# zuds-survey/zuds-pipeline

Hardware: AMD Instinct MI355X
Metric: Mpix/s resample->coadd->subtract, 3072x3072 frames (higher is better)
Workload: dtype f32; 1 GPU; configs[1]+[2]: 32x 3072x3072 TPV frames/GPU, mesh background + weight rescale + Lanczos-3 resample + WEIGHTED coadd (+ AND mask coadd, int16 masks); then 1 science frame/GPU: align ref, hotpants 3x3 regions x 10x10 stamps, r=10, ko=4, subtract; frames_per_gpu=32, size=3072, mask_dtype=int16, combine=WEIGHTED, subtract=True

## Files before the change

zuds-pipeline_amd/csrc/hotpants.hip:

```cpp
#include "hp_dev.h"
#include <sched.h>
#include "chol_diag.h"

static __device__ __forceinline__ void hp_zero_words(int* __restrict__ zero0, int nzero0, int* __restrict__ zero1, int nzero1) {
    if (blockIdx.x != 0) return;
    if (zero0) for (int k = threadIdx.x; k < nzero0; k += blockDim.x) zero0[k] = 0;
    if (zero1) for (int k = threadIdx.x; k < nzero1; k += blockDim.x) zero1[k] = 0;
}
__global__ void k_hp_valid(const float* __restrict__ sci, const float* __restrict__ ref,
                           const uint8_t* __restrict__ bpm, int64_t n, float il, float iu,
                           float tl, float tu, uint8_t* __restrict__ bad,
                           const double* __restrict__ lim, double nsig,
                           int* __restrict__ zero0 = nullptr, int nzero0 = 0,
                           int* __restrict__ zero1 = nullptr, int nzero1 = 0) {
    int64_t p = (int64_t)blockIdx.x * blockDim.x + threadIdx.x;
    hp_zero_words(zero0, nzero0, zero1, nzero1);
    if (lim) {
        il = (float)(lim[0] - nsig * lim[1]);
        tl = (float)(lim[3] - nsig * lim[4]);
    }
    if (p >= n) return;
    float s = sci[p], t = ref[p];
    bool ok = (s == s) && (t == t) && fabsf(s) < 3e38f && fabsf(t) < 3e38f;
    ok = ok && s >= il && s <= iu && t >= tl && t <= tu;
// ... 67 lines not shown
        if (lane == 0) wsum[4 * c + wave] = __popcll(m);
    }
    if (tid == 0) ra_pre[0] = 0;
    __syncthreads();
    {
        const int v = tid < 4 * nch ? wsum[tid] : 0;
        int inc = v;
#pragma unroll
        for (int o = 1; o < 64; o <<= 1) {
            const int t = __shfl_up(inc, o);
            if (lane >= o) inc += t;
        }
        if (lane == 63) wtot[wave] = inc;
        __syncthreads();
        int off = inc - v;
        for (int w = 0; w < wave; ++w) off += wtot[w];
        if (tid < 4 * nch) wsum[tid] = off;
    }
    __syncthreads();
    for (int c = 0; c < nch; ++c) {
        const int x = 256 * c + tid;
        if (x < nx) ra_pre[x + 1] += wsum[4 * c + wave];
    }
    __syncthreads();
    for (int x = tid; x < nx; x += 256) {
        const int a1 = max(x - hw1, 0), b1 = min(x + hw1, nx - 1);
        const int a2 = max(x - hw2, 0), b2 = min(x + hw2, nx - 1);
        out1[r0 + x] = (ra_pre[b1 + 1] - ra_pre[a1]) > 0;
        out2[r0 + x] = (ra_pre[b2 + 1] - ra_pre[a2]) > 0;
    }
}

#define HP_COLSTRIP 96
__global__ __launch_bounds__(256) void k_hp_colany(const uint8_t* __restrict__ in, int nx, int ny, int hw,
                                                   int edge, uint8_t* __restrict__ out) {
    const int x = blockIdx.x * blockDim.x + threadIdx.x;
    const int y0 = blockIdx.y * HP_COLSTRIP, y1 = min(y0 + HP_COLSTRIP, ny);
    if (x >= nx) return;
    int cnt = 0;
    for (int j = max(y0 - hw, 0); j <= min(y0 + hw, ny - 1); ++j) cnt += in[(size_t)j * nx + x] ? 1 : 0;
    for (int y = y0; y < y1; ++y) {
        uint8_t v = cnt > 0;
        if (edge && (x < hw || x >= nx - hw || y < hw || y >= ny - hw)) v = 1;
        out[(size_t)y * nx + x] = v;
        const int add = y + 1 + hw, sub = y - hw;
        if (add < ny) cnt += in[(size_t)add * nx + x] ? 1 : 0;
        if (sub >= 0) cnt -= in[(size_t)sub * nx + x] ? 1 : 0;
    }
}

#define HP_COLSTRIP4 32
__global__ __launch_bounds__(256) void k_hp_colany4(const uint8_t* __restrict__ in, int nx, int ny, int hw,
                                                    int edge, uint8_t* __restrict__ out) {
    const int x = (blockIdx.x * blockDim.x + threadIdx.x) * 4;
    const int y0 = blockIdx.y * HP_COLSTRIP4, y1 = min(y0 + HP_COLSTRIP4, ny);
    if (x >= nx) return;
    const unsigned* in4 = reinterpret_cast<const unsigned*>(in + x);
    const size_t pitch = (size_t)nx / 4;
    auto nz = [](unsigned w, int k) -> int { return ((w >> (8 * k)) & 0xffu) ? 1 : 0; };
    int cnt[4] = {0, 0, 0, 0};
    {
        const int j0 = max(y0 - hw, 0), j1 = min(y0 + hw, ny - 1);
        for (int jb = j0; jb <= j1; jb += 8) {
            unsigned w[8];
#pragma unroll
            for (int u = 0; u < 8; ++u) w[u] = (jb + u <= j1) ? in4[(size_t)(jb + u) * pitch] : 0u;
#pragma unroll
            for (int u = 0; u < 8; ++u)
#pragma unroll
                for (int k = 0; k < 4; ++k) cnt[k] += nz(w[u], k);
        }
    }
    for (int yb = y0; yb < y1; yb += 8) {
        unsigned wa[8], ws[8];
#pragma unroll
        for (int u = 0; u < 8; ++u) {
            const int add = yb + u + 1 + hw, sub = yb + u - hw;
            wa[u] = (add < ny) ? in4[(size_t)add * pitch] : 0u;
            ws[u] = (sub >= 0) ? in4[(size_t)sub * pitch] : 0u;
        }
#pragma unroll
        for (int u = 0; u < 8; ++u) {
            const int y = yb + u;
            if (y < y1) {
                unsigned o = 0;
#pragma unroll
                for (int k = 0; k < 4; ++k) {
                    unsigned v = cnt[k] > 0;
                    if (edge && (x + k < hw || x + k >= nx - hw || y < hw || y >= ny - hw)) v = 1;
                    o |= v << (8 * k);
                }
                *reinterpret_cast<unsigned*>(out + (size_t)y * nx + x) = o;
            }
#pragma unroll
            for (int k = 0; k < 4; ++k) cnt[k] += nz(wa[u], k) - nz(ws[u], k);
        }
    }
}

__global__ __launch_bounds__(256) void k_hp_cells(const hp_plan P, const float* __restrict__ ref,
                                                  const uint8_t* __restrict__ bad,
                                                  const uint8_t* __restrict__ dirty,
                                                  int2* __restrict__ centres) {
    __shared__ double red[4];
    __shared__ float bval[4];
    __shared__ int bidx[4];
    __shared__ int2 chosen[HP_MAXNSS];
    const int cell = blockIdx.x, tid = threadIdx.x;
    const int r = cell / P.ncellr, c = cell - r * P.ncellr;
    const int sy = c / P.nsx, sx = c - sy * P.nsx;
    const int cw = (P.rx1[r] - P.rx0[r]) / P.nsx, ch = (P.ry1[r] - P.ry0[r]) / P.nsy;
    const int cx0 = P.rx0[r] + sx * cw, cy0 = P.ry0[r] + sy * ch;
    const int n = cw * ch;
    double m = 0.0, s = 0.0;
    for (int pass = 0; pass < 4; ++pass) {
        double s0 = 0, s1 = 0;
        for (int k = tid; k < n; k += 256) {
            int yy = k / cw, xx = k - yy * cw;
            size_t idx = (size_t)(cy0 + yy) * P.nx + cx0 + xx;
            if (bad[idx]) continue;
            double v = ref[idx];
            if (pass == 0 || fabs(v - m) <= 3.0 * s) { s0 += 1.0; s1 += v; }
        }
        s0 = block_sum256(s0, red);
        s1 = block_sum256(s1, red);
        if (s0 < 1.0) break;
        double mn = s1 / s0;
        double s2 = 0;
        for (int k = tid; k < n; k += 256) {
            int yy = k / cw, xx = k - yy * cw;
            size_t idx = (size_t)(cy0 + yy) * P.nx + cx0 + xx;
            if (bad[idx]) continue;
            double v = ref[idx];
            if (pass == 0 || fabs(v - m) <= 3.0 * s) s2 += (v - mn) * (v - mn);
        }
        s2 = block_sum256(s2, red);
        m = mn;
        s = sqrt(s2 / s0);
    }
    const double thr = m + P.ft * s;
    for (int k = 0; k < P.nss; ++k) {
        float best = -__builtin_inff();
        int bi = 0x7fffffff;
        for (int q = tid; q < n; q += 256) {
            int yy = q / cw, xx = q - yy * cw;
            int x = cx0 + xx, y = cy0 + yy;
            size_t idx = (size_t)y * P.nx + x;
            if (dirty[idx]) continue;
            float v = ref[idx];
            if (!((double)v >= thr)) continue;
            bool excl = false;
            for (int e = 0; e < k; ++e)
                excl |= (abs(x - chosen[e].x) <= P.hwss) && (abs(y - chosen[e].y) <= P.hwss);
            if (excl) continue;
            if (v > best || (v == best && q < bi)) { best = v; bi = q; }
        }
#pragma unroll
        for (int o = 32; o >= 1; o >>= 1) {
            float ov = __shfl_xor(best, o);
            int oi = __shfl_xor(bi, o);
            if (ov > best || (ov == best && oi < bi)) { best = ov; bi = oi; }
        }
        __syncthreads();
        if ((tid & 63) == 0) { bval[tid >> 6] = best; bidx[tid >> 6] = bi; }
        __syncthreads();
        if (tid == 0) {
            for (int w = 1; w < 4; ++w)
                if (bval[w] > best || (bval[w] == best && bidx[w] < bi)) { best = bval[w]; bi = bidx[w]; }
            int2 cc = make_int2(-1, -1);
            if (bi != 0x7fffffff) { int yy = bi / cw; cc = make_int2(cx0 + bi - yy * cw, cy0 + yy); }
            chosen[k] = cc;
            centres[cell * P.nss + k] = cc;
        }
        __syncthreads();
        if (chosen[k].x < 0) {
            if (tid == 0)
                for (int e = k + 1; e < P.nss; ++e) centres[cell * P.nss + e] = make_int2(-1, -1);
            break;
        }
    }
}

#define HC_PX 24
#define HC_THREADS 512
__global__ __launch_bounds__(HC_THREADS, 4) void k_hp_cells_reg(const hp_plan P, const float* __restrict__ ref,
                                                      const uint8_t* __restrict__ bad,
                                                      const uint8_t* __restrict__ dirty,
                                                      int2* __restrict__ centres) {
    __shared__ double red[HC_THREADS / 64];
    __shared__ float bval[HC_THREADS / 64];
    __shared__ int bidx[HC_THREADS / 64];
    __shared__ int2 chosen[HP_MAXNSS];
    const int cell = blockIdx.x, tid = threadIdx.x;
    const int r = cell / P.ncellr, c = cell - r * P.ncellr;
    const int sy = c / P.nsx, sx = c - sy * P.nsx;
    const int cw = (P.rx1[r] - P.rx0[r]) / P.nsx, ch = (P.ry1[r] - P.ry0[r]) / P.nsy;
    const int cx0 = P.rx0[r] + sx * cw, cy0 = P.ry0[r] + sy * ch;
    const int n = cw * ch;
    const int dyy = HC_THREADS / cw, dxx = HC_THREADS - dyy * cw;
    const int yy0 = tid / cw, xx0 = tid - yy0 * cw;
    float v[HC_PX];
    unsigned long long okm = 0, cleanm = 0;
    {
        int yy = yy0, xx = xx0;
#pragma unroll
        for (int i = 0; i < HC_PX; ++i) {
            const int k = tid + HC_THREADS * i;
            float val = 0.f;
            if (k < n) {
                const size_t idx = (size_t)(cy0 + yy) * P.nx + cx0 + xx;
                val = ref[idx];
                if (!bad[idx]) okm |= 1ull << i;
                if (!dirty[idx]) cleanm |= 1ull << i;
            }
            v[i] = val;
            xx += dxx; yy += dyy;
            if (xx >= cw) { xx -= cw; ++yy; }
        }
    }
    double m = 0.0, s = 0.0;
    for (int pass = 0; pass < 4; ++pass) {
        double s0 = 0, s1 = 0;
#pragma unroll
        for (int i = 0; i < HC_PX; ++i) {
            float vf = v[i];
            asm volatile("" : "+v"(vf));
            const double vv = vf;
            if ((okm >> i & 1) && (pass == 0 || fabs(vv - m) <= 3.0 * s)) { s0 += 1.0; s1 += vv; }
        }
        s0 = block_sum_waves<HC_THREADS / 64>(s0, red);
        s1 = block_sum_waves<HC_THREADS / 64>(s1, red);
        if (s0 < 1.0) break;
        const double mn = s1 / s0;
        double s2 = 0;
#pragma unroll
        for (int i = 0; i < HC_PX; ++i) {
            float vf = v[i];
            asm volatile("" : "+v"(vf));
            const double vv = vf;
            if ((okm >> i & 1) && (pass == 0 || fabs(vv - m) <= 3.0 * s)) s2 += (vv - mn) * (vv - mn);
        }
        s2 = block_sum_waves<HC_THREADS / 64>(s2, red);
        m = mn;
        s = sqrt(s2 / s0);
    }
    const double thr = m + P.ft * s;
    unsigned long long cand = 0;
#pragma unroll
    for (int i = 0; i < HC_PX; ++i)
        if ((cleanm >> i & 1) && ((double)v[i] >= thr)) cand |= 1ull << i;
    int2 last = make_int2(-1000000, -1000000);
    for (int k = 0; k < P.nss; ++k) {
        float best = -__builtin_inff();
        int bi = 0x7fffffff;
        {
            int yy = yy0, xx = xx0;
            asm volatile("" : "+v"(yy), "+v"(xx));
#pragma unroll
            for (int i = 0; i < HC_PX; ++i) {
                if (cand >> i & 1) {
                    const int x = cx0 + xx, y = cy0 + yy, q = tid + HC_THREADS * i;
                    const bool excl = (abs(x - last.x) <= P.hwss) && (abs(y - last.y) <= P.hwss);
                    if (excl) cand &= ~(1ull << i);
                    else if (v[i] > best || (v[i] == best && q < bi)) { best = v[i]; bi = q; }
                }
                xx += dxx; yy += dyy;
                if (xx >= cw) { xx -= cw; ++yy; }
            }
        }
#pragma unroll
        for (int o = 32; o >= 1; o >>= 1) {
            float ov = __shfl_xor(best, o);
            int oi = __shfl_xor(bi, o);
            if (ov > best || (ov == best && oi < bi)) { best = ov; bi = oi; }
        }
        __syncthreads();
        if ((tid & 63) == 0) { bval[tid >> 6] = best; bidx[tid >> 6] = bi; }
        __syncthreads();
        if (tid == 0) {
            for (int w = 1; w < HC_THREADS / 64; ++w)
                if (bval[w] > best || (bval[w] == best && bidx[w] < bi)) { best = bval[w]; bi = bidx[w]; }
            int2 cc = make_int2(-1, -1);
            if (bi != 0x7fffffff) { int yy = bi / cw; cc = make_int2(cx0 + bi - yy * cw, cy0 + yy); }
            chosen[k] = cc;
            centres[cell * P.nss + k] = cc;
        }
        __syncthreads();
        last = chosen[k];
        if (last.x < 0) {
            if (tid == 0)
                for (int e = k + 1; e < P.nss; ++e) centres[cell * P.nss + e] = make_int2(-1, -1);
            break;
        }
    }
}


typedef double double4_t __attribute__((ext_vector_type(4)));

#define GR_KT 32
#define GR_PITCH 34

#define GR_SPLIT 8
static __device__ __forceinline__ void hp_gram_body(const hp_plan& P, const double* __restrict__ X,
                                                 const int* __restrict__ need,
                                                 const int* __restrict__ active,
                                                 double* __restrict__ Gp, const int* __restrict__ guard,
                                                 const int* __restrict__ list) {
    if (guard && *guard == 0) return;
    __shared__ double L[HP_MAXX * GR_PITCH];
    const int tid = threadIdx.x;
    const int ncl = list ? list[0] : (int)gridDim.x;
#pragma unroll 1
    for (int ci = blockIdx.x; ci < ncl; ci += gridDim.x) {
    const int cell = list ? list[1 + ci] : ci;
    __syncthreads();
    if (!need[cell] || active[cell] < 0) continue;
    const double* Xc = X + (size_t)cell * P.nX * P.npixp;
    const int wave = tid >> 6, lane = tid & 63;
    const int li = lane & 15, lk = lane >> 4;
    const int ntile = P.npixp / GR_KT;
    const int per = (ntile + GR_SPLIT - 1) / GR_SPLIT;
    const int kbeg = blockIdx.y * per * GR_KT, kend = min((int)(blockIdx.y + 1) * per, ntile) * GR_KT;
    double4_t acc[4];
#pragma unroll
    for (int c = 0; c < 4; ++c) acc[c] = (double4_t){0.0, 0.0, 0.0, 0.0};
    constexpr int GR_LD = HP_MAXX * GR_KT / 256;
    double nxt[GR_LD];
    auto fetch = [&](int k0) {
#pragma unroll
        for (int q = 0; q < GR_LD; ++q) {
            const int e = tid + 256 * q, row = e >> 5, col = e & 31;
            nxt[q] = row < P.nX ? Xc[(size_t)row * P.npixp + k0 + col] : 0.0;
        }
    };
    if (kbeg < kend) fetch(kbeg);
    for (int k0 = kbeg; k0 < kend; k0 += GR_KT) {
        __syncthreads();
#pragma unroll
        for (int q = 0; q < GR_LD; ++q) {
            const int e = tid + 256 * q, row = e >> 5, col = e & 31;
            L[row * GR_PITCH + col] = nxt[q];
        }
        __syncthreads();
        if (k0 + GR_KT < kend) fetch(k0 + GR_KT);
#pragma unroll
        for (int kk = 0; kk < GR_KT / 4; ++kk) {
            double a = L[(16 * wave + li) * GR_PITCH + 4 * kk + lk];
#pragma unroll
            for (int c = 0; c < 4; ++c) {
                double b = L[(16 * c + li) * GR_PITCH + 4 * kk + lk];
                acc[c] = __builtin_amdgcn_mfma_f64_16x16x4f64(a, b, acc[c], 0, 0, 0);
            }
        }
    }
    double* Gc = Gp + ((size_t)cell * GR_SPLIT + blockIdx.y) * HP_MAXX * HP_MAXX;
#pragma unroll
    for (int c = 0; c < 4; ++c)
#pragma unroll
        for (int rg = 0; rg < 4; ++rg)
            Gc[(size_t)(16 * wave + lk + 4 * rg) * HP_MAXX + 16 * c + li] = acc[c][rg];
    }
}

#define GS_THREADS 1024
static __device__ __forceinline__ void hp_gram_sum_body(const double* __restrict__ Gp,
                                                     const int* __restrict__ need,
                                                     const int* __restrict__ active,
                                                     double* __restrict__ G, const int* __restrict__ guard,
                                                     double* __restrict__ Gold, const int* __restrict__ list) {
    if (guard && *guard == 0) return;
    const int ncl = list ? list[0] : (int)gridDim.x;
    constexpr int NE = HP_MAXX * HP_MAXX / GS_THREADS;
#pragma unroll 1
    for (int ci = blockIdx.x; ci < ncl; ci += gridDim.x) {
        const int cell = list ? list[1 + ci] : ci;
        if (!need[cell] || active[cell] < 0) continue;
        const double* src = Gp + (size_t)cell * GR_SPLIT * HP_MAXX * HP_MAXX;
        double* dst = G + (size_t)cell * HP_MAXX * HP_MAXX;
        double* old = Gold ? Gold + (size_t)cell * HP_MAXX * HP_MAXX : nullptr;
        double part[NE][GR_SPLIT], prev[NE];
#pragma unroll
        for (int q = 0; q < NE; ++q) {
            const int e = threadIdx.x + GS_THREADS * q;
#pragma unroll
            for (int sl = 0; sl < GR_SPLIT; ++sl) part[q][sl] = src[(size_t)sl * HP_MAXX * HP_MAXX + e];
            prev[q] = old ? dst[e] : 0.0;
        }
#pragma unroll
        for (int q = 0; q < NE; ++q) {
            const int e = threadIdx.x + GS_THREADS * q;
            double v = 0.0;
#pragma unroll
            for (int sl = 0; sl < GR_SPLIT; ++sl) v += part[q][sl];
            if (old) old[e] = prev[q];
            dst[e] = v;
        }
    }
}

__device__ inline void col_decode(const hp_plan& P, int c, int* n, int* p) {
    if (c == 0) { *n = 0; *p = -1; return; }
    int k = c - 1;
    if (k < (P.nc - 1) * P.nkp) { *n = 1 + k / P.nkp; *p = k % P.nkp; return; }
    *n = P.nc + (k - (P.nc - 1) * P.nkp);
    *p = -1;
}

__global__ __launch_bounds__(256) void k_hp_build(const hp_plan P, const double* __restrict__ G,
                                                  const double* __restrict__ phi,
                                                  const int* __restrict__ active,
                                                  const int* __restrict__ chg, int sign,
                                                  double* __restrict__ A,
                                                  double* __restrict__ rhs, const int* __restrict__ guard,
                                                  unsigned* __restrict__ zero = nullptr, int nzero = 0) {
    if (guard && *guard == 0) return;
    const int reg = blockIdx.z;
    if (zero && blockIdx.x == 0 && blockIdx.y == 0)
        for (int k = threadIdx.x; k < nzero; k += 256) zero[(size_t)reg * nzero + k] = 0u;
    const int c1 = blockIdx.y * 16 + (threadIdx.x >> 4), c2 = blockIdx.x * 16 + (threadIdx.x & 15);
    if (blockIdx.x > blockIdx.y) return;
    if (c1 >= P.nunk || c2 >= P.nunk) return;
    int n1, p1, n2, p2;
    col_decode(P, c1, &n1, &p1);
    col_decode(P, c2, &n2, &p2);
    double acc = 0.0, racc = 0.0;
    const bool do_rhs = (c2 == 0);
    bool any = false;
    const int* list = chg + P.ncell + reg * (P.ncellr + 1);
    const int ncand = (sign == 0) ? P.ncellr : list[0];
    for (int s0 = 0; s0 < ncand; s0 += 8) {
        double g[8], gr[8], w1[8], w2[8];
        bool on[8];
#pragma unroll
        for (int u = 0; u < 8; ++u) {
            const int s = s0 + u;
            on[u] = false;
            g[u] = gr[u] = 0.0;
            w1[u] = w2[u] = 1.0;
            if (s < ncand) {
                const int cell = (sign == 0) ? reg * P.ncellr + s : list[1 + s];
                on[u] = !(active[cell] < 0 && sign >= 0);
                if (on[u]) {
                    const double* Gc = G + (size_t)cell * HP_MAXX * HP_MAXX;
                    const double* ph = phi + (size_t)cell * P.nkp;
                    if (p1 >= 0) w1[u] = ph[p1];
                    if (p2 >= 0) w2[u] = ph[p2];
                    g[u] = Gc[n1 * HP_MAXX + n2];
                    if (do_rhs) gr[u] = Gc[n1 * HP_MAXX + P.nE];
                }
            }
        }
#pragma unroll
        for (int u = 0; u < 8; ++u)
            if (on[u]) {
                any = true;
                acc += w1[u] * w2[u] * g[u];
                if (do_rhs) racc += w1[u] * gr[u];
            }
    }
    const size_t ia = (size_t)reg * (size_t)(P.nunk + 1) * P.nunk + (size_t)c1 * P.nunk + c2;
    if (sign == 0) {
        if (c2 <= c1) A[ia] = acc;
        if (do_rhs) rhs[(size_t)reg * P.nunk + c1] = racc;
    } else if (any) {
        if (c2 <= c1) A[ia] += sign * acc;
        if (do_rhs) rhs[(size_t)reg * P.nunk + c1] += sign * racc;
    }
}

#define BB_CH 128
#define HBB_PAIRS 5
#define BU_CH 32
#define BB_LDS (BB_CH * 18 + BB_CH / 2)
static __device__ __forceinline__ void hp_pair_decode(const int pair, int* n1o, int* n2o) {
    int n1 = (int)((sqrtf(8.f * (float)pair + 1.f) - 1.f) * 0.5f);
    while (n1 * (n1 + 1) / 2 > pair) --n1;
    while ((n1 + 1) * (n1 + 2) / 2 <= pair) ++n1;
    *n1o = n1;
    *n2o = pair - n1 * (n1 + 1) / 2;
}
static __device__ __forceinline__ void hp_blk_entry_add(const double w1, const double w2, const double g, const double gr,
                                                     const bool do_rhs, double& acc, double& racc) {
    acc += w1 * w2 * g;
    if (do_rhs) racc += w1 * gr;
}
static __device__ __forceinline__ void hp_build_blk_body(const int reg, const int pair, const hp_plan& P, const double* __restrict__ G,
                                                      const double* __restrict__ phi,
                                                      const int* __restrict__ active,
                                                      double* __restrict__ A,
                                                      double* __restrict__ rhs,
                                                      unsigned* __restrict__ zero, int nzero, double* sh) {
    int n1, n2;
    hp_pair_decode(pair, &n1, &n2);
    if (zero && n1 == 0 && n2 == 0)
        for (int k = threadIdx.x; k < nzero; k += 256) zero[(size_t)reg * nzero + k] = 0u;
    const int p1 = threadIdx.x >> 4, p2 = threadIdx.x & 15;
    const bool k1 = n1 >= 1 && n1 < P.nc, k2 = n2 >= 1 && n2 < P.nc;
    const int nk = (P.nc - 1) * P.nkp;
    const int c1 = n1 == 0 ? 0 : (k1 ? 1 + (n1 - 1) * P.nkp + p1 : 1 + nk + (n1 - P.nc));
    const int c2 = n2 == 0 ? 0 : (k2 ? 1 + (n2 - 1) * P.nkp + p2 : 1 + nk + (n2 - P.nc));
    const bool live = p1 < (k1 ? P.nkp : 1) && p2 < (k2 ? P.nkp : 1) && c2 <= c1;
    const bool do_rhs = (c2 == 0);
    double *gs = sh, *grs = sh + BB_CH, *phs = sh + 2 * BB_CH;
    int* ons = reinterpret_cast<int*>(sh + 18 * BB_CH);
    const int tid = threadIdx.x;
    const size_t ia = (size_t)reg * (size_t)(P.nunk + 1) * P.nunk + (size_t)c1 * P.nunk + c2;
    double acc = 0.0, racc = 0.0;
    for (int s0 = 0; s0 < P.ncellr; s0 += BB_CH) {
        const int nch = min(BB_CH, P.ncellr - s0);
        __syncthreads();
        if (tid < nch) {
            const int cell = reg * P.ncellr + s0 + tid;
            const int on = active[cell] >= 0;
            const double* Gc = G + (size_t)cell * HP_MAXX * HP_MAXX;
            ons[tid] = on;
            gs[tid] = on ? Gc[n1 * HP_MAXX + n2] : 0.0;
            grs[tid] = (on && n2 == 0) ? Gc[n1 * HP_MAXX + P.nE] : 0.0;
        }
        for (int e = tid; e < nch * P.nkp; e += 256) {
            const int k = e / P.nkp, pp = e - k * P.nkp;
            phs[k * 16 + pp] = phi[(size_t)(reg * P.ncellr + s0 + k) * P.nkp + pp];
        }
        __syncthreads();
        if (live) {
            for (int k = 0; k < nch; ++k) {
                if (!ons[k]) continue;
                const double w1 = k1 ? phs[k * 16 + p1] : 1.0, w2 = k2 ? phs[k * 16 + p2] : 1.0;
                hp_blk_entry_add(w1, w2, gs[k], do_rhs ? grs[k] : 0.0, do_rhs, acc, racc);
            }
        }
    }
    if (!live) return;
    A[ia] = acc;
    if (do_rhs) rhs[(size_t)reg * P.nunk + c1] = racc;
}

static __device__ __forceinline__ void hp_update_blk_body(const int reg, const int pair0, const hp_plan& P, const double* __restrict__ G,
                                                       const double* __restrict__ phi, const int* __restrict__ active,
                                                       const int* __restrict__ chg, double* __restrict__ A,
                                                       double* __restrict__ rhs, unsigned* __restrict__ zero, int nzero,
                                                       const double* __restrict__ Gold, const double* __restrict__ phiold,
                                                       const int* __restrict__ need, double* sh) {
    static_assert(HBB_PAIRS * BU_CH <= 256 && BU_CH * 16 == 512, "one Gram item and two spatial-term items per thread");
    static_assert(4 * HBB_PAIRS * BU_CH + 2 * BU_CH * 16 + BU_CH <= BB_LDS, "the update's staging fits the build's LDS");
    double (*ug)[HBB_PAIRS][BU_CH] = reinterpret_cast<double (*)[HBB_PAIRS][BU_CH]>(sh);
    double (*ugr)[HBB_PAIRS][BU_CH] = reinterpret_cast<double (*)[HBB_PAIRS][BU_CH]>(sh + 2 * HBB_PAIRS * BU_CH);
    double (*uph)[BU_CH * 16] = reinterpret_cast<double (*)[BU_CH * 16]>(sh + 4 * HBB_PAIRS * BU_CH);
    int* uon = reinterpret_cast<int*>(sh + 4 * HBB_PAIRS * BU_CH + 2 * BU_CH * 16);
    const int tid = threadIdx.x;
    const int npair = P.nE * (P.nE + 1) / 2;
    if (zero && pair0 == 0)
        for (int k = tid; k < nzero; k += 256) zero[(size_t)reg * nzero + k] = 0u;
    const int* list = chg + P.ncell + reg * (P.ncellr + 1);
    const int ncand = list[0];
    if (ncand <= 0) return;
    const int p1 = tid >> 4, p2 = tid & 15;
    const int nk = (P.nc - 1) * P.nkp;
    bool k1[HBB_PAIRS], k2[HBB_PAIRS], live[HBB_PAIRS], do_rhs[HBB_PAIRS], any1[HBB_PAIRS];
    size_t ia[HBB_PAIRS], ir[HBB_PAIRS];
    double av[HBB_PAIRS], rv[HBB_PAIRS], acc0[HBB_PAIRS], racc0[HBB_PAIRS], acc1[HBB_PAIRS], racc1[HBB_PAIRS];
    {
        int n1, n2;
        hp_pair_decode(pair0, &n1, &n2);
#pragma unroll
        for (int q = 0; q < HBB_PAIRS; ++q) {
            k1[q] = n1 >= 1 && n1 < P.nc;
            k2[q] = n2 >= 1 && n2 < P.nc;
            const int c1 = n1 == 0 ? 0 : (k1[q] ? 1 + (n1 - 1) * P.nkp + p1 : 1 + nk + (n1 - P.nc));
            const int c2 = n2 == 0 ? 0 : (k2[q] ? 1 + (n2 - 1) * P.nkp + p2 : 1 + nk + (n2 - P.nc));
            live[q] = pair0 + q < npair && p1 < (k1[q] ? P.nkp : 1) && p2 < (k2[q] ? P.nkp : 1) && c2 <= c1;
            do_rhs[q] = (c2 == 0);
            ia[q] = (size_t)reg * (size_t)(P.nunk + 1) * P.nunk + (size_t)c1 * P.nunk + c2;
            ir[q] = (size_t)reg * P.nunk + c1;
            any1[q] = false;
            av[q] = rv[q] = acc0[q] = racc0[q] = acc1[q] = racc1[q] = 0.0;
            if (live[q]) {
                av[q] = A[ia[q]];
                if (do_rhs[q]) rv[q] = rhs[ir[q]];
            }
            if (++n2 > n1) { ++n1; n2 = 0; }
        }
    }
    const int gq = min(tid / BU_CH, HBB_PAIRS - 1), gk = tid % BU_CH;
    const bool gdo = tid < HBB_PAIRS * BU_CH && pair0 + gq < npair;
    int gn1, gn2;
    hp_pair_decode(min(pair0 + gq, npair - 1), &gn1, &gn2);
    for (int s0 = 0; s0 < ncand; s0 += BU_CH) {
        const int nch = min(BU_CH, ncand - s0);
        __syncthreads();
        {
            const int cg = list[1 + s0 + min(gk, nch - 1)];
            int cp[2], pp[2];
#pragma unroll
            for (int u = 0; u < 2; ++u) {
                const int e = tid + 256 * u;
                cp[u] = list[1 + s0 + min(e >> 4, nch - 1)];
                pp[u] = min(e & 15, P.nkp - 1);
            }
            const int wasg = need[cg], ong = active[cg] >= 0;
            const double* Gn = G + (size_t)cg * HP_MAXX * HP_MAXX;
            const double* Go = Gold + (size_t)cg * HP_MAXX * HP_MAXX;
            const double gnew = Gn[gn1 * HP_MAXX + gn2], gold = Go[gn1 * HP_MAXX + gn2];
            const double rnew = Gn[gn1 * HP_MAXX + P.nE], rold = Go[gn1 * HP_MAXX + P.nE];
            int wasp[2];
            double fnew[2], fold[2];
#pragma unroll
            for (int u = 0; u < 2; ++u) {
                wasp[u] = need[cp[u]];
                fnew[u] = phi[(size_t)cp[u] * P.nkp + pp[u]];
                fold[u] = phiold[(size_t)cp[u] * P.nkp + pp[u]];
            }
            if (gdo && gk < nch) {
                ug[0][gq][gk] = wasg ? gold : gnew;
                ugr[0][gq][gk] = gn2 == 0 ? (wasg ? rold : rnew) : 0.0;
                ug[1][gq][gk] = ong ? gnew : 0.0;
                ugr[1][gq][gk] = (ong && gn2 == 0) ? rnew : 0.0;
                if (gq == 0) uon[gk] = ong;
            }
#pragma unroll
            for (int u = 0; u < 2; ++u) {
                const int e = tid + 256 * u;
                if ((e >> 4) < nch && (e & 15) < P.nkp) {
                    uph[0][e] = wasp[u] ? fold[u] : fnew[u];
                    uph[1][e] = fnew[u];
                }
            }
        }
        __syncthreads();
        for (int k = 0; k < nch; ++k) {
            const double f1o = uph[0][k * 16 + p1], f2o = uph[0][k * 16 + p2];
            const double f1n = uph[1][k * 16 + p1], f2n = uph[1][k * 16 + p2];
            const bool back = uon[k] != 0;
#pragma unroll
            for (int q = 0; q < HBB_PAIRS; ++q)
                if (live[q]) {
                    hp_blk_entry_add(k1[q] ? f1o : 1.0, k2[q] ? f2o : 1.0, ug[0][q][k], do_rhs[q] ? ugr[0][q][k] : 0.0,
                                     do_rhs[q], acc0[q], racc0[q]);
                    if (back) {
                        any1[q] = true;
                        hp_blk_entry_add(k1[q] ? f1n : 1.0, k2[q] ? f2n : 1.0, ug[1][q][k], do_rhs[q] ? ugr[1][q][k] : 0.0,
                                         do_rhs[q], acc1[q], racc1[q]);
                    }
                }
        }
    }
#pragma unroll
    for (int q = 0; q < HBB_PAIRS; ++q)
        if (live[q]) {
            av[q] += -1.0 * acc0[q];
            if (do_rhs[q]) rv[q] += -1.0 * racc0[q];
            if (any1[q]) {
                av[q] += acc1[q];
                if (do_rhs[q]) rv[q] += racc1[q];
            }
            A[ia[q]] = av[q];
            if (do_rhs[q]) rhs[ir[q]] = rv[q];
        }
}

#define BM_CH 128
static __device__ __forceinline__ void hp_build_mfma_body(const hp_plan& P, const double* __restrict__ G,
                                                       const double* __restrict__ phi, const int* __restrict__ active,
                                                       double* __restrict__ A, double* __restrict__ rhs,
                                                       unsigned* __restrict__ zero, int nzero) {
    typedef double bm_double4 __attribute__((ext_vector_type(4)));
// ... 2638 lines not shown
```

zuds-pipeline_amd/csrc/hp_vectors.hip:

```cpp
#include "hp_dev.h"

template <int HWK, bool BIG = false>
static __device__ __forceinline__ void hp_vectors_body(const hp_plan& P, const float* __restrict__ sci,
                                                    const float* __restrict__ ref,
                                                    const float* __restrict__ srms,
                                                    const float* __restrict__ trms,
                                                    const double* __restrict__ filt,
                                                    const int2* __restrict__ centres,
                                                    const int* __restrict__ active,
                                                    const int* __restrict__ need,
                                                    double* __restrict__ X,
                                                    double* __restrict__ phi,
                                                    double* __restrict__ vbar, const int* __restrict__ guard,
                                                    double* __restrict__ phiold, const int* __restrict__ list,
                                                    int special, int cwarg = 0, double* __restrict__ w0g = nullptr) {
    if (guard && *guard == 0) return;
    extern __shared__ double hp_smem[];
    constexpr int STEP = 2 * HWK + 1;
    constexpr int WIN = HV_R + 2 * HWK;
    const int tid = threadIdx.x;
    const int part = blockIdx.y, nparts = gridDim.y;
    const int ncl = list ? list[0] : (BIG ? P.ncell : (int)gridDim.x);
#pragma unroll 1
    for (int ci = blockIdx.x; ci < ncl; ci += gridDim.x) {
    const int cell = list ? list[1 + ci] : ci;
    __syncthreads();
    if (!need[cell]) continue;
    const int act = active[cell];
    if (act < 0) continue;
    const int2 cc = centres[cell * P.nss + act];
    const int r = cell / P.ncellr;
    const int pw = P.pw, sw = P.sw, hwss = P.hwss;
    const bool only_special = special && part == 0;
    const int fpart = special ? part - 1 : part, fparts = special ? nparts - 1 : nparts;
    const int pp = pw + HV_R;
    const int cw = BIG ? cwarg : P.sw;
    double* xp = hp_smem;
    double* w0 = (BIG && w0g) ? w0g + ((size_t)blockIdx.y * gridDim.x + blockIdx.x) * (size_t)P.npix
                              : xp + (size_t)(pw + HV_R) * cw;
    double* red = (BIG && w0g) ? xp + (size_t)(pw + HV_R) * cw : w0 + P.npix;
    float* patch = reinterpret_cast<float*>(red + 8);
    for (int k0 = tid; !only_special && k0 < pw * pw; k0 += HV_THREADS * 10) {
        float t[10];
#pragma unroll
        for (int u = 0; u < 10; ++u) {
            const int k = k0 + HV_THREADS * u;
            const int yy = k / pw, xx = k - yy * pw;
            t[u] = (k < pw * pw) ? ref[(size_t)(cc.y - P.hw + yy) * P.nx + (cc.x - P.hw + xx)] : 0.f;
        }
#pragma unroll
        for (int u = 0; u < 10; ++u) {
            const int k = k0 + HV_THREADS * u;
            const int yy = k / pw, xx = k - yy * pw;
            if (k < pw * pw) patch[yy * pp + xx] = t[u];
        }
    }
#pragma clang loop vectorize(disable) interleave(disable) unroll(disable)
    for (int k = tid; k < pw * HV_R; k += HV_THREADS) patch[(k / HV_R) * pp + pw + k % HV_R] = 0.f;
#pragma clang loop vectorize(disable) interleave(disable) unroll(disable)
    for (int k = tid; k < HV_R * cw; k += HV_THREADS) xp[(size_t)pw * cw + k] = 0.0;
    const double xc = P.rx0[r] + 0.5 * (P.rx1[r] - P.rx0[r]), hx = 0.5 * (P.rx1[r] - P.rx0[r]);
    const double yc = P.ry0[r] + 0.5 * (P.ry1[r] - P.ry0[r]), hy = 0.5 * (P.ry1[r] - P.ry0[r]);
    double* Xc = X + (size_t)cell * P.nX * P.npixp;
    double vs = 0.0;
    for (int k0 = tid; part == 0 && tid < 256 && k0 < P.npixp; k0 += 256 * 5) {
        float ts[5], ta[5], tb[5];
#pragma unroll
        for (int u = 0; u < 5; ++u) {
            const int k = k0 + 256 * u;
            ts[u] = ta[u] = tb[u] = 0.f;
            if (k < P.npix) {
                const int i = k / sw, j = k - i * sw;
                const size_t idx = (size_t)(cc.y - hwss + i) * P.nx + (cc.x - hwss + j);
                ts[u] = sci[idx];
                ta[u] = srms[idx];
                tb[u] = trms[idx];
            }
        }
#pragma unroll
        for (int u = 0; u < 5; ++u) {
            int k = k0 + 256 * u;
            asm volatile("" : "+v"(k));
            if (k < P.npix) {
                const int i = k / sw, j = k - i * sw;
                const int x = cc.x - hwss + j, y = cc.y - hwss + i;
                Xc[(size_t)P.nE * P.npixp + k] = (double)ts[u];
                const double a = ta[u], b = tb[u];
                vs += a * a + b * b;
                const double xf = (x - xc) / hx, yf = (y - yc) / hy;
                for (int q = 0; q < P.nbg; ++q)
                    Xc[(size_t)(P.nc + q) * P.npixp + k] = ipowd(xf, P.bpi[q]) * ipowd(yf, P.bpj[q]);
            } else if (k < P.npixp) {
                for (int q = 0; q < P.nX; ++q) Xc[(size_t)q * P.npixp + k] = 0.0;
            }
        }
    }
    vs = block_sum_waves<HV_THREADS / 64>(vs, red);
    if (tid == 0 && part == 0) {
        vbar[cell] = vs / P.npix;
        double fx = (cc.x - xc) / hx, fy = (cc.y - yc) / hy;
        if (phiold) {
#pragma clang loop vectorize(disable) interleave(disable) unroll(disable)
            for (int p = 0; p < P.nkp; ++p) phiold[(size_t)cell * P.nkp + p] = phi[(size_t)cell * P.nkp + p];
        }
#pragma clang loop vectorize(disable) interleave(disable) unroll(disable)
        for (int p = 0; p < P.nkp; ++p)
            phi[(size_t)cell * P.nkp + p] = ipowd(fx, P.kpi[p]) * ipowd(fy, P.kpj[p]);
    }
    __syncthreads();
    if (only_special) continue;
    const int nstrip = (sw + HV_R - 1) / HV_R;
    int fidx = 0;
    for (int f = 0; f < P.nf1; ++f) {
        const int tn0 = P.tf0[f], tn1 = tn0 + P.tfn[f];
        if (tn1 == tn0) continue;
        const bool mine = (fidx % fparts) == fpart;
        ++fidx;
        const bool for_w0 = (P.tfx[0] == f);
        if (!mine && !for_w0) continue;
        const double* fxv = filt + f * STEP;
        const int nchunks = BIG ? (sw + cw - 1) / cw : 1;
        for (int ch = 0; ch < nchunks; ++ch) {
        const int c0 = BIG ? ch * cw : 0;
        const int cwe = BIG ? min(cw, sw - c0) : sw;
        const int nstripc = BIG ? (cwe + HV_R - 1) / HV_R : nstrip;
        for (int e = tid; e < pw * nstripc; e += HV_THREADS) {
            const int yy = e / nstripc, jl0 = (e - yy * nstripc) * HV_R, j0 = c0 + jl0;
            const float* pr = patch + yy * pp + j0;
            double wv[WIN];
#pragma unroll
            for (int k = 0; k < WIN; ++k) wv[k] = (double)pr[k];
            double acc[HV_R];
#pragma unroll
            for (int q = 0; q < HV_R; ++q) acc[q] = 0.0;
#pragma unroll
            for (int m = 0; m < STEP; ++m) {
                const double cf = fxv[2 * HWK - m];
#pragma unroll
                for (int q = 0; q < HV_R; ++q) acc[q] += cf * wv[q + m];
            }
#pragma unroll
            for (int q = 0; q < HV_R; ++q)
                if (j0 + q < sw) xp[yy * cw + jl0 + q] = acc[q];
        }
        __syncthreads();
        for (int n = tn0; n < tn1; ++n) {
            if (!mine && n != 0) continue;
            const double* fyv = filt + P.tfy[n] * STEP;
            const double sc = P.tscale[n];
            const bool sub0 = n != 0 && P.tsub0[n] != 0;
            for (int e = tid; e < cwe * nstrip; e += HV_THREADS) {
                const int s = e / cwe, jl = e - s * cwe, j = c0 + jl;
                const int i0 = s * HV_R;
                const double* col = xp + i0 * cw + jl;
                double wv[WIN];
#pragma unroll
                for (int k = 0; k < WIN; ++k) wv[k] = col[k * cw];
                double acc[HV_R];
#pragma unroll
                for (int q = 0; q < HV_R; ++q) acc[q] = 0.0;
#pragma unroll
                for (int m = 0; m < STEP; ++m) {
                    const double cf = fyv[2 * HWK - m];
#pragma unroll
                    for (int q = 0; q < HV_R; ++q) acc[q] += cf * wv[q + m];
                }
                double wsub[HV_R];
#pragma unroll
                for (int q = 0; q < HV_R; ++q) wsub[q] = 0.0;
                if (sub0) {
#pragma unroll
                    for (int q = 0; q < HV_R; ++q) wsub[q] = w0[min(i0 + q, sw - 1) * sw + j];
                }
#pragma unroll
                for (int q = 0; q < HV_R; ++q) {
                    const int i = i0 + q;
                    const int k = i * sw + j;
                    const double v = acc[q] * sc - wsub[q];
                    if (i < sw) {
                        if (n == 0) w0[k] = v;
                        if (mine) Xc[(size_t)n * P.npixp + k] = v;
                    }
                }
            }
            if (n == 0) __syncthreads();
        }
        __syncthreads();
        }
    }
    }
}

template <int HWK>
__global__ __launch_bounds__(HV_THREADS) void k_hp_vectors(const hp_plan P, const float* __restrict__ sci,
                                                    const float* __restrict__ ref, const float* __restrict__ srms,
                                                    const float* __restrict__ trms, const double* __restrict__ filt,
                                                    const int2* __restrict__ centres, const int* __restrict__ active,
                                                    const int* __restrict__ need, double* __restrict__ X,
                                                    double* __restrict__ phi, double* __restrict__ vbar,
                                                    const int* __restrict__ guard, double* __restrict__ phiold,
                                                    const int* __restrict__ list, int special) {
    hp_vectors_body<HWK>(P, sci, ref, srms, trms, filt, centres, active, need, X, phi, vbar, guard, phiold, list, special);
}
template <int HWK>
__global__ __launch_bounds__(HV_THREADS) void k_hp_vectors_big(const hp_plan P, const float* __restrict__ sci,
                                                    const float* __restrict__ ref, const float* __restrict__ srms,
                                                    const float* __restrict__ trms, const double* __restrict__ filt,
                                                    const int2* __restrict__ centres, const int* __restrict__ active,
                                                    const int* __restrict__ need, double* __restrict__ X,
                                                    double* __restrict__ phi, double* __restrict__ vbar,
                                                    const int* __restrict__ guard, double* __restrict__ phiold,
                                                    const int* __restrict__ list, int special, int cw, double* __restrict__ w0g) {
    hp_vectors_body<HWK, true>(P, sci, ref, srms, trms, filt, centres, active, need, X, phi, vbar, guard, phiold, list, special,
                               cw, w0g);
}
template <int HWK>
__global__ __launch_bounds__(HV_THREADS, (HWK <= 11 ? 4 : 2)) void k_hp_vectors_b(const hp_plan P, const hp_job* __restrict__ jobs,
                                                      const double* __restrict__ filt, int round) {
    const hp_job& J = jobs[blockIdx.z];
    hp_vectors_body<HWK>(P, J.sci, J.ref, J.srms, J.trms, filt, J.centres, J.active, J.need, J.X, J.phi, J.vbar,
                         HPJ_GUARD(J, round), J.phiold, round > 1 ? J.needlist : nullptr, round > 1 ? 1 : 0);
}


int zm_hp_launch_vectors(zm_ctx* ctx, hipStream_t st, const hp_plan& P, const hv_cfg& hvc, int rounds, int ncl_grid, int hv_gx,
                         const float* sci, const float* ref, const float* sci_rms, const float* ref_rms, const double* d_filt,
                         const int2* centres, const int* active, const int* need, double* X, double* phi, double* vbar,
                         const int* guard, double* phiold, const int* needlist, double* hv_w0g) {
    const size_t vsh = hvc.shmem;
    const dim3 grid_s(rounds == 1 ? P.ncell : ncl_grid, rounds == 1 ? HV_SPLIT_ALL : HV_SPLIT_FEW);
    const dim3 grid_b(rounds == 1 ? hv_gx : std::min(ncl_grid, hv_gx), rounds == 1 ? HV_SPLIT_ALL : HV_SPLIT_FEW);
    const int* list = rounds == 1 ? nullptr : needlist;
    const int special = rounds == 1 ? 0 : 1;
    if (hvc.big) {
#define C(H) case H: \
    ZM_HIP(hipFuncSetAttribute((const void*)k_hp_vectors_big<H>, hipFuncAttributeMaxDynamicSharedMemorySize, (int)vsh)); \
    hipLaunchKernelGGL(k_hp_vectors_big<H>, grid_b, dim3(HV_THREADS), vsh, st, P, sci, ref, sci_rms, ref_rms, d_filt, \
                       centres, active, need, X, phi, vbar, guard, phiold, list, special, hvc.cw, hv_w0g); break;
        switch (P.hwk) {
            C(1) C(2) C(3) C(4) C(5) C(6) C(7) C(8) C(9) C(10) C(11) C(12) C(13) C(14) C(15) C(16) C(17) C(18) C(19) C(20)
            default: zm_set_error("zm_subtract: unsupported kernel half width %d", P.hwk); return 2;
        }
#undef C
    } else {
#define C(H) case H: \
    ZM_HIP(hipFuncSetAttribute((const void*)k_hp_vectors<H>, hipFuncAttributeMaxDynamicSharedMemorySize, (int)vsh)); \
    hipLaunchKernelGGL(k_hp_vectors<H>, grid_s, dim3(HV_THREADS), vsh, st, P, sci, ref, sci_rms, ref_rms, d_filt, \
                       centres, active, need, X, phi, vbar, guard, phiold, list, special); break;
        switch (P.hwk) {
            C(1) C(2) C(3) C(4) C(5) C(6) C(7) C(8) C(9) C(10) C(11) C(12) C(13) C(14) C(15) C(16) C(17) C(18) C(19) C(20)
            default: zm_set_error("zm_subtract: unsupported kernel half width %d", P.hwk); return 2;
        }
#undef C
    }
    ZM_HIP(hipGetLastError());
    return 0;
}

int zm_hp_launch_vectors_b(zm_ctx* ctx, hipStream_t st, const hp_plan& P, size_t vsh, unsigned gcells, unsigned NJ,
                           const hp_job* d_tab, const double* d_filt, int round) {
#define C(H) case H: \
    ZM_HIP(hipFuncSetAttribute((const void*)k_hp_vectors_b<H>, hipFuncAttributeMaxDynamicSharedMemorySize, (int)vsh)); \
    hipLaunchKernelGGL(k_hp_vectors_b<H>, dim3(gcells, round == 1 ? HV_SPLIT_ALL : HV_SPLIT_FEW, NJ), dim3(HV_THREADS), vsh, st, \
                       P, d_tab, d_filt, round); break;
    switch (P.hwk) {
        C(1) C(2) C(3) C(4) C(5) C(6) C(7) C(8) C(9) C(10) C(11) C(12) C(13) C(14) C(15)
        default: zm_set_error("zm_subtract: unsupported kernel half width %d", P.hwk); return 2;
    }
#undef C
    return 0;
}
```

Before: 50140 Mpix/s.

## Exploit Gram symmetry in MFMA tiles and retune hotpants vector y-pass

Result: faster. 50900 Mpix/s (median of 6 runs) (+1.5%).

```diff
diff --git a/zuds-pipeline_amd/csrc/hotpants.hip b/zuds-pipeline_amd/csrc/hotpants.hip
--- a/zuds-pipeline_amd/csrc/hotpants.hip
+++ b/zuds-pipeline_amd/csrc/hotpants.hip
@@ -393,6 +393,31 @@
 #define GR_PITCH 34
 
 #define GR_SPLIT 8
+template <int NT, int R0, int C0, int R1, int C1, int R2, int C2>
+static __device__ __forceinline__ void hp_gram_ktile(const double* L, int li, int lk, double4_t (&acc)[3]) {
+#pragma unroll
+    for (int kk = 0; kk < GR_KT / 4; ++kk) {
+        const double* Lk = L + li * GR_PITCH + 4 * kk + lk;
+        acc[0] = __builtin_amdgcn_mfma_f64_16x16x4f64(Lk[16 * R0 * GR_PITCH], Lk[16 * C0 * GR_PITCH], acc[0], 0, 0, 0);
+        if (NT > 1) acc[1] = __builtin_amdgcn_mfma_f64_16x16x4f64(Lk[16 * R1 * GR_PITCH], Lk[16 * C1 * GR_PITCH], acc[1], 0, 0, 0);
+        if (NT > 2) acc[2] = __builtin_amdgcn_mfma_f64_16x16x4f64(Lk[16 * R2 * GR_PITCH], Lk[16 * C2 * GR_PITCH], acc[2], 0, 0, 0);
+    }
+}
+template <int R, int C>
+static __device__ __forceinline__ void hp_gram_store(double* Gc, int li, int lk, const double4_t& a) {
+#pragma unroll
+    for (int rg = 0; rg < 4; ++rg) {
+        Gc[(size_t)(16 * R + lk + 4 * rg) * HP_MAXX + 16 * C + li] = a[rg];
+        if (R != C) Gc[(size_t)(16 * C + li) * HP_MAXX + 16 * R + lk + 4 * rg] = a[rg];
+    }
+}
+#define GR_DEAL(sel, F) \
+    switch (sel) { \
+        case 0: F(3, 3, 0, 3, 1, 3, 2) break; \
+        case 1: F(3, 2, 0, 2, 1, 2, 2) break; \
+        case 2: F(2, 1, 0, 1, 1, 0, 0) break; \
+        default: F(2, 0, 0, 3, 3, 0, 0) break; \
+    }
 static __device__ __forceinline__ void hp_gram_body(const hp_plan& P, const double* __restrict__ X,
                                                  const int* __restrict__ need,
                                                  const int* __restrict__ active,
@@ -410,12 +435,13 @@
     const double* Xc = X + (size_t)cell * P.nX * P.npixp;
     const int wave = tid >> 6, lane = tid & 63;
     const int li = lane & 15, lk = lane >> 4;
+    const int sel = __builtin_amdgcn_readfirstlane((wave + blockIdx.x + blockIdx.y) & 3);
     const int ntile = P.npixp / GR_KT;
     const int per = (ntile + GR_SPLIT - 1) / GR_SPLIT;
     const int kbeg = blockIdx.y * per * GR_KT, kend = min((int)(blockIdx.y + 1) * per, ntile) * GR_KT;
-    double4_t acc[4];
-#pragma unroll
-    for (int c = 0; c < 4; ++c) acc[c] = (double4_t){0.0, 0.0, 0.0, 0.0};
+    double4_t acc[3];
+#pragma unroll
+    for (int c = 0; c < 3; ++c) acc[c] = (double4_t){0.0, 0.0, 0.0, 0.0};
     constexpr int GR_LD = HP_MAXX * GR_KT / 256;
     double nxt[GR_LD];
     auto fetch = [&](int k0) {
@@ -435,24 +461,20 @@
         }
         __syncthreads();
         if (k0 + GR_KT < kend) fetch(k0 + GR_KT);
-#pragma unroll
-        for (int kk = 0; kk < GR_KT / 4; ++kk) {
-            double a = L[(16 * wave + li) * GR_PITCH + 4 * kk + lk];
-#pragma unroll
-            for (int c = 0; c < 4; ++c) {
-                double b = L[(16 * c + li) * GR_PITCH + 4 * kk + lk];
-                acc[c] = __builtin_amdgcn_mfma_f64_16x16x4f64(a, b, acc[c], 0, 0, 0);
-            }
-        }
+#define GR_STEP(NT, R0, C0, R1, C1, R2, C2) hp_gram_ktile<NT, R0, C0, R1, C1, R2, C2>(L, li, lk, acc);
+        GR_DEAL(sel, GR_STEP)
+#undef GR_STEP
     }
     double* Gc = Gp + ((size_t)cell * GR_SPLIT + blockIdx.y) * HP_MAXX * HP_MAXX;
-#pragma unroll
-    for (int c = 0; c < 4; ++c)
-#pragma unroll
-        for (int rg = 0; rg < 4; ++rg)
-            Gc[(size_t)(16 * wave + lk + 4 * rg) * HP_MAXX + 16 * c + li] = acc[c][rg];
-    }
-}
+#define GR_OUT(NT, R0, C0, R1, C1, R2, C2) { \
+        hp_gram_store<R0, C0>(Gc, li, lk, acc[0]); \
+        if (NT > 1) hp_gram_store<R1, C1>(Gc, li, lk, acc[1]); \
+        if (NT > 2) hp_gram_store<R2, C2>(Gc, li, lk, acc[2]); }
+    GR_DEAL(sel, GR_OUT)
+#undef GR_OUT
+    }
+}
+#undef GR_DEAL
 
 #define GS_THREADS 1024
 static __device__ __forceinline__ void hp_gram_sum_body(const double* __restrict__ Gp,
diff --git a/zuds-pipeline_amd/csrc/hp_vectors.hip b/zuds-pipeline_amd/csrc/hp_vectors.hip
--- a/zuds-pipeline_amd/csrc/hp_vectors.hip
+++ b/zuds-pipeline_amd/csrc/hp_vectors.hip
@@ -1,4 +1,66 @@
 #include "hp_dev.h"
+
+static __device__ __forceinline__ void hv_pin(double (&a)[8]) {
+    asm volatile("" : "+v"(a[0]), "+v"(a[1]), "+v"(a[2]), "+v"(a[3]), "+v"(a[4]), "+v"(a[5]), "+v"(a[6]), "+v"(a[7]));
+}
+static __device__ __forceinline__ void hv_pin(double (&a)[5]) {
+    asm volatile("" : "+v"(a[0]), "+v"(a[1]), "+v"(a[2]), "+v"(a[3]), "+v"(a[4]));
+}
+
+#define HV_RY 5
+static __device__ __forceinline__ int hv_rows_y(int cwe, int sw) {
+    return (cwe * ((sw + HV_R - 1) / HV_R) > HV_THREADS / 2 && cwe * ((sw + HV_RY - 1) / HV_RY) <= HV_THREADS) ? HV_RY : HV_R;
+}
+
+template <int HWK, int R, bool PIN>
+static __device__ __forceinline__ void hv_ypass(int tid, int cwe, int c0, int sw, const double* xp, int cw,
+                                             const double* __restrict__ fyv, double sc, bool sub0, bool first, bool mine,
+                                             double* w0, char* Xn) {
+    constexpr int STEP = 2 * HWK + 1, WIN = R + 2 * HWK;
+    const unsigned rowb = (unsigned)sw * (unsigned)sizeof(double);
+    const unsigned cwb = (unsigned)cw * (unsigned)sizeof(double);
+    const int nstrip = (sw + R - 1) / R;
+    for (int e = tid; e < cwe * nstrip; e += HV_THREADS) {
+        const int s = e / cwe, jl = e - s * cwe, j = c0 + jl;
+        const int i0 = s * R;
+        unsigned colb = (unsigned)(i0 * cw + jl) * (unsigned)sizeof(double);
+        if (PIN) asm volatile("" : "+v"(colb));
+        const char* col = reinterpret_cast<const char*>(xp) + colb;
+        double wv[WIN];
+#pragma unroll
+        for (int k = 0; k < WIN; ++k)
+            wv[k] = *reinterpret_cast<const double*>(col + (unsigned)k * cwb);
+        double acc[R];
+#pragma unroll
+        for (int q = 0; q < R; ++q) acc[q] = 0.0;
+#pragma unroll
+        for (int m = 0; m < STEP; ++m) {
+            const double cf = fyv[2 * HWK - m];
+#pragma unroll
+            for (int q = 0; q < R; ++q) acc[q] += cf * wv[q + m];
+        }
+        hv_pin(acc);
+        int k0 = i0 * sw + j;
+        asm volatile("" : "+v"(k0));
+        const int nv = sw - i0;
+        double wsub[R];
+#pragma unroll
+        for (int q = 0; q < R; ++q) wsub[q] = 0.0;
+        if (sub0) {
+            const int klast = (sw - 1) * sw + j;
+#pragma unroll
+            for (int q = 0; q < R; ++q) wsub[q] = w0[min(k0 + q * sw, klast)];
+        }
+#pragma unroll
+        for (int q = 0; q < R; ++q) {
+            const double v = acc[q] * sc - wsub[q];
+            if (q < nv) {
+                if (first) w0[k0 + q * sw] = v;
+                if (mine) *reinterpret_cast<double*>(Xn + ((unsigned)k0 * (unsigned)sizeof(double) + q * rowb)) = v;
+            }
+        }
+    }
+}
 
 template <int HWK, bool BIG = false>
 static __device__ __forceinline__ void hp_vectors_body(const hp_plan& P, const float* __restrict__ sci,
@@ -139,9 +201,12 @@
 #pragma unroll
                 for (int q = 0; q < HV_R; ++q) acc[q] += cf * wv[q + m];
             }
+            hv_pin(acc);
+            double* xo = xp + yy * cw + jl0;
+            const int nv = sw - j0;
 #pragma unroll
             for (int q = 0; q < HV_R; ++q)
-                if (j0 + q < sw) xp[yy * cw + jl0 + q] = acc[q];
+                if (q < nv) xo[q] = acc[q];
         }
         __syncthreads();
         for (int n = tn0; n < tn1; ++n) {
@@ -149,40 +214,12 @@
             const double* fyv = filt + P.tfy[n] * STEP;
             const double sc = P.tscale[n];
             const bool sub0 = n != 0 && P.tsub0[n] != 0;
-            for (int e = tid; e < cwe * nstrip; e += HV_THREADS) {
-                const int s = e / cwe, jl = e - s * cwe, j = c0 + jl;
-                const int i0 = s * HV_R;
-                const double* col = xp + i0 * cw + jl;
-                double wv[WIN];
-#pragma unroll
-                for (int k = 0; k < WIN; ++k) wv[k] = col[k * cw];
-                double acc[HV_R];
-#pragma unroll
-                for (int q = 0; q < HV_R; ++q) acc[q] = 0.0;
-#pragma unroll
-                for (int m = 0; m < STEP; ++m) {
-                    const double cf = fyv[2 * HWK - m];
-#pragma unroll
-                    for (int q = 0; q < HV_R; ++q) acc[q] += cf * wv[q + m];
-                }
-                double wsub[HV_R];
-#pragma unroll
-                for (int q = 0; q < HV_R; ++q) wsub[q] = 0.0;
-                if (sub0) {
-#pragma unroll
-                    for (int q = 0; q < HV_R; ++q) wsub[q] = w0[min(i0 + q, sw - 1) * sw + j];
-                }
-#pragma unroll
-                for (int q = 0; q < HV_R; ++q) {
-                    const int i = i0 + q;
-                    const int k = i * sw + j;
-                    const double v = acc[q] * sc - wsub[q];
-                    if (i < sw) {
-                        if (n == 0) w0[k] = v;
-                        if (mine) Xc[(size_t)n * P.npixp + k] = v;
-                    }
-                }
-            }
+            char* Xn = reinterpret_cast<char*>(Xc + (size_t)n * P.npixp);
+            constexpr bool PIN = !BIG && HWK <= 15;
+            if (!BIG && hv_rows_y(cwe, sw) == HV_RY)
+                hv_ypass<HWK, HV_RY, PIN>(tid, cwe, c0, sw, xp, cw, fyv, sc, sub0, n == 0, mine, w0, Xn);
+            else
+                hv_ypass<HWK, HV_R, PIN>(tid, cwe, c0, sw, xp, cw, fyv, sc, sub0, n == 0, mine, w0, Xn);
             if (n == 0) __syncthreads();
         }
         __syncthreads();
```
